# holoskii/Rendering

Measured on AMD Instinct MI355X. Metric: Mrays/s + ms/frame at 4096^2, 250k-tri BVH scene, higher is better.
Workload: dtype f32

## Files before the change

### rendering_amd/csrc/rtx_kernels.hip

```cpp
#include <hip/hip_runtime.h>
#include <stdint.h>

#include "rtx_device.h"
#include "rtx_tuning.h"

#pragma clang fp contract(off)

using namespace rtxd;

constexpr uint32_t kPopNum = 1u, kPopDen = 2u;

namespace {

#if RTX_DBG
#define RTX_DBG_ONLY(...) __VA_ARGS__
#else
#define RTX_DBG_ONLY(...)
#endif
#if RTX_DBG || RTX_WAVE_TRACE
#define RTX_TRACE_ONLY(...) __VA_ARGS__
#else
#define RTX_TRACE_ONLY(...)
#endif

// ... 1094 lines not shown
	s.li = 0; s.si = 0; s.dsum = 0; s.ssum = 0;
}

struct LightRec { int type; V3 color; float intensity; V3 dir, pos; uint32_t nPoints; const float* points; };

template <bool PLAIN = false>
__device__ __forceinline__ void advance(const Params& P, Lane& s, uint32_t gl)
{
	const int maxDepth = P.view.maxDepth;
	const float bias = P.view.bias;
	V3& col = PLAIN ? s.diff : s.col;
	bool run = true;
	do {
		if (!run) continue;
		if (s.state == ST_NEWRAY) {
			RTX_T0
			if (s.sp > maxDepth) { col = skyColor(P, s.rd); s.state = ST_RETURN; RTX_ACC(0) continue; }
			s.qtmax = kFltMax;
			s.state = ST_WAIT_PRIMARY;
			run = false; continue;
		}
		if (s.state == ST_NEXT_LIGHT) {
			RTX_T0
			if (s.li >= P.nLights) { s.state = ST_LIGHTS_DONE; continue; }
			const uint32_t li0 = __builtin_amdgcn_readfirstlane(s.li);
			uint32_t liS = li0;
			if (PLAIN) asm volatile("" : "+s"(liS));
			if (s.li != li0) continue;
			LightRec lr;
			{
				const u32x16 w = sload16(P.lights + liS);
				lr.type = (int)w[0]; lr.color = mk(F(w[1]), F(w[2]), F(w[3])); lr.intensity = F(w[4]);
				lr.dir = mk(F(w[5]), F(w[6]), F(w[7])); lr.pos = mk(F(w[8]), F(w[9]), F(w[10])); lr.nPoints = w[11];
				lr.points = (const float*)(((uint64_t)w[13] << 32) | w[12]);
			}
			const LightRec* l = &lr;
			const int lt = l->type;
			if (PLAIN && lt != 1 && lt != 2) __builtin_unreachable();
			float dist;
			if (lt == 1) {
				s.L = l->dir;
				s.I = l->color * l->intensity;
				dist = kFltMax;
			}
			else if (lt == 2) {
				const V3 lp = l->pos;
				V3 L = s.P - lp;
				s.I = l->color * attenuation(l->intensity, len2(L));
				s.L = normalized(L);
				dist = length(s.P - lp);
			}
			else {
				const uint32_t np = l->nPoints;
				if (s.si == 0) {
					const V3 lp = l->pos;
					s.I = l->color * attenuation(l->intensity, len2(s.P - lp));
					s.dsum = 0; s.ssum = 0;
				}
				if (s.si >= np) {
					const float fn = (float)np;
					if (s.mat == 0) s.diff = s.diff + s.I * (s.dsum / fn);
					else if (s.mat == 3) {
						s.diff = s.diff + s.I * (s.dsum / fn);
						s.spec = s.spec + s.I * powfRef(s.ssum / fn, s.nSpec);
					}
					else s.spec = s.spec + s.I * powfRef(s.ssum / fn, s.nSpec);
					s.li++; s.si = 0;
					continue;
				}
				V3 L = s.P - load3(inGlobal(l->points) + (size_t)s.si * 3);
				dist = length(L);
				s.L = normalized(L);
			}
			s.qmoot = s.mat == 0 && fmaxRef(0.f, dot(s.N, -s.L)) == 0.f;
			s.qarea = lt == 3;
			s.qsrc = (lt == 2 && liS < P.nSrcLights && len2(s.N) <= P.srcNmax2) ? 2u + liS : 0u;
			s.qtmax = dist;
			s.state = ST_WAIT_SHADOW;
			RTX_ACC(1)
			run = false; continue;
		}
		if (s.state == ST_LIGHTS_DONE) {
			RTX_T0
			const Object* ob = P.objects + s.obj;
			if (PLAIN && s.mat != 0) __builtin_unreachable();
			if (s.mat == 0) { col = s.objColor * s.diff; s.state = ST_RETURN; continue; }
			if (s.mat == 3) {
				s.col = s.objColor * ob->ambient + s.diff * ob->diffuse + s.spec * s.specCoef;
				s.state = ST_RETURN; continue;
			}
			if (s.mat == 1) {
				frameAt(P, gl, s.sp, 0) = __int_as_float(FR_REFL);
				frameAt(P, gl, s.sp, 2) = s.spec.x; frameAt(P, gl, s.sp, 3) = s.spec.y; frameAt(P, gl, s.sp, 4) = s.spec.z;
				const V3 nd = s.rd - s.N * (2 * dot(s.rd, s.N));
				s.ro = s.P + s.N * bias; s.rd = nd;
				s.sp++; s.state = ST_NEWRAY; RTX_ACC(2) continue;
			}
			const float ior = ob->ior;
			const float kr = fresnelKr(s.rd, s.N, ior);
			const bool outside = dot(s.rd, s.N) < 0;
			const V3 biasVec = s.N * bias;
			const V3 fd = normalized(reflectDir(s.rd, s.N));
			const V3 fo = outside ? s.P + biasVec : s.P - biasVec;
			frameAt(P, gl, s.sp, 1) = kr;
			frameAt(P, gl, s.sp, 2) = s.spec.x; frameAt(P, gl, s.sp, 3) = s.spec.y; frameAt(P, gl, s.sp, 4) = s.spec.z;
			if (kr < 1) {
				const V3 rd = normalized(refractDir(s.rd, s.N, ior));
				const V3 ro = outside ? s.P - biasVec : s.P + biasVec;
				frameAt(P, gl, s.sp, 0) = __int_as_float(FR_TRANS1);
				frameAt(P, gl, s.sp, 8) = fo.x; frameAt(P, gl, s.sp, 9) = fo.y; frameAt(P, gl, s.sp, 10) = fo.z;
				frameAt(P, gl, s.sp, 11) = fd.x; frameAt(P, gl, s.sp, 12) = fd.y; frameAt(P, gl, s.sp, 13) = fd.z;
				s.ro = ro; s.rd = rd;
			}
			else {
				frameAt(P, gl, s.sp, 0) = __int_as_float(FR_TRANS2);
				frameAt(P, gl, s.sp, 5) = 0.f; frameAt(P, gl, s.sp, 6) = 0.f; frameAt(P, gl, s.sp, 7) = 0.f;
				s.ro = fo; s.rd = fd;
			}
			s.sp++; s.state = ST_NEWRAY; RTX_ACC(3) continue;
		}
		if (s.state == ST_RETURN) {
			RTX_T0
			if (s.sp == 0) { s.state = ST_DONE; run = false; continue; }
			if (PLAIN) __builtin_unreachable();
			s.sp--;
			float fr[kFrameFields];
			for (int k = 0; k < kFrameFields; ++k) fr[k] = frameAt(P, gl, s.sp, k);
			asm volatile("" : "+v"(fr[0]), "+v"(fr[1]), "+v"(fr[2]), "+v"(fr[3]), "+v"(fr[4]), "+v"(fr[5]), "+v"(fr[6]));
			asm volatile("" : "+v"(fr[7]), "+v"(fr[8]), "+v"(fr[9]), "+v"(fr[10]), "+v"(fr[11]), "+v"(fr[12]), "+v"(fr[13]));
			const int kind = __float_as_int(fr[0]);
			const V3 spec = mk(fr[2], fr[3], fr[4]);
			if (kind == FR_REFL) { s.col = s.col * 0.8f + spec; RTX_ACC(4) continue; }
			const float kr = fr[1];
			if (kind == FR_TRANS1) {
				const V3 acc = mk(0, 0, 0) + s.col * (1 - kr);
				frameAt(P, gl, s.sp, 0) = __int_as_float(FR_TRANS2);
				frameAt(P, gl, s.sp, 5) = acc.x; frameAt(P, gl, s.sp, 6) = acc.y; frameAt(P, gl, s.sp, 7) = acc.z;
				s.ro = mk(fr[8], fr[9], fr[10]);
				s.rd = mk(fr[11], fr[12], fr[13]);
				s.sp++; s.state = ST_NEWRAY; RTX_ACC(5) continue;
			}
			V3 acc = mk(fr[5], fr[6], fr[7]);
			acc = acc + s.col * kr;
			s.col = acc + spec * kr;
			RTX_ACC(6)
			continue;
		}
		run = false;
	} while (ballot(run) != 0);
}

template <bool PLAIN = false>
__device__ __forceinline__ void consume(const Params& P, Lane& s, const Hit& h)
{
	if (s.state == ST_WAIT_PRIMARY) {
		RTX_T0
		if (h.obj < 0) { (PLAIN ? s.diff : s.col) = skyColor(P, s.rd); s.state = ST_RETURN; RTX_ACC(7) return; }
		shadePrimary(P, s, h);
		if (PLAIN) s.mat = 0;
		s.state = ST_NEXT_LIGHT;
		RTX_ACC(8)
		return;
	}
	if (s.state == ST_WAIT_SHADOW) {
		RTX_T0
		const float vis = (h.obj < 0) ? 1.0f : 0.0f;
		if (PLAIN && (s.mat != 0 || s.qarea)) __builtin_unreachable();
		const bool area = s.qarea;
		const V3 nL = -s.L;
		if (s.mat == 0) {
			const float c = vis * fmaxRef(0.f, dot(s.N, nL));
			if (!area) s.diff = s.diff + s.I * c;
			else s.dsum += c;
		}
		else {
			const V3 R = reflectDir(s.L, s.N);
			const float sd = fmaxRef(0.f, dot(R, -s.rd));
			if (!area) {
				const V3 vI = s.I * vis;
				if (s.mat == 3) s.diff = s.diff + vI * fmaxRef(0.f, dot(s.N, nL));
				s.spec = s.spec + vI * powfRef(sd, s.nSpec);
			}
			else {
				if (s.mat == 3) s.dsum += vis * fmaxRef(0.f, dot(s.N, nL));
				s.ssum += vis * sd;
			}
		}
		if (area) s.si++; else s.li++;
		s.state = ST_NEXT_LIGHT;
		RTX_ACC(9)
	}
}

__device__ __forceinline__ void primaryRay(const Params& P, float x, float y, V3& o, V3& d)
{
	const float w = (float)P.view.width, hgt = (float)P.view.height;
	const float xp = (2 * (x + 0.5f) / w - 1) * P.view.scale * P.view.aspect;
	const float yp = -(2 * (y + 0.5f) / hgt - 1) * P.view.scale;
	const V3 s = normalized(mk(xp, yp, -1));
	const float* M = P.view.camM;
	V3 r;
	r.x = s.x * M[0] + s.y * M[4] + s.z * M[8] + M[12];
	r.y = s.x * M[1] + s.y * M[5] + s.z * M[9] + M[13];
	r.z = s.x * M[2] + s.y * M[6] + s.z * M[10] + M[14];
	const float ww = s.x * M[3] + s.y * M[7] + s.z * M[11] + M[15];
	if (ww != 0.0f && ww != 1.0f) { const float wi = 1.0f / ww; r.x *= wi; r.y *= wi; r.z *= wi; }
	o = mk(P.view.camPos[0], P.view.camPos[1], P.view.camPos[2]);
	d = r;
}

constexpr int kParkFields = 25;
template <bool PLAIN> struct ParkLayout { static constexpr int kFields = kParkFields - (PLAIN ? 4 : 0), kSp = PLAIN ? -3 : 0; };
template <bool PLAIN>
__device__ __forceinline__ float (*parkArea())[256]
{
	__shared__ float area[ParkLayout<PLAIN>::kFields][256];
	return area;
}
static_assert(sizeof(powTab) + sizeof(leafBatch) + sizeof(wideStack) + sizeof(pruneUni) + ParkLayout<false>::kFields * 1024 <= (RTX_WAVES >= 5 ? 31744 : 40960),
              "the ray kernels' LDS no longer fits the blocks per CU that RTX_WAVES asks for");
static_assert(RTX_WAVES_PLAIN < 6 || sizeof(leafBatch) + sizeof(wideStack) + sizeof(pruneUni) + ParkLayout<true>::kFields * 1024 <= 27136,
              "the PLAIN kernels' LDS no longer fits six blocks per CU (160 KB / 6, rounded down to the allocation granule)");

__device__ __forceinline__ const Params& freshParams(const Params& P)
{
	uint64_t p = (uint64_t)(uintptr_t)__builtin_amdgcn_kernarg_segment_ptr();
	asm volatile("" : "+s"(p));
	return *(const Params*)(const RTX_AS4 Params*)p;
}

template <bool STATS, bool MESH = true, bool FEWRAYS = false, bool BOXES = true, bool CAM = true, int CULLK = -1, bool PLAIN = false>
__device__ __forceinline__ V3 castRayWave(const Params& P0, bool valid, V3 o, V3 d, uint32_t gl, Counts& cnt)
{
	const Params& P = freshParams(P0);
	Lane s;
	s.state = valid ? ST_NEWRAY : ST_DONE;
	s.sp = 0; s.ro = o; s.rd = d; s.col = mk(0, 0, 0);
	s.obj = 0; s.mat = 0; s.li = 0; s.si = 0;
	s.P = s.N = s.objColor = s.diff = s.spec = s.L = s.I = mk(0, 0, 0);
	s.specCoef = s.nSpec = s.dsum = s.ssum = 0;
	s.qtmax = kFltMax; s.qmoot = false; s.qarea = false; s.qsrc = 0;
	RTX_DBG_ONLY(unsigned long long dbgRounds = 0, dbgTrace = 0, dbgState = 0;)
	for (;;) {
		advance<PLAIN>(freshParams(P0), s, gl);
		if (ballot(s.state != ST_DONE) == 0) break;
		Hit h;
		RTX_DBG_ONLY(const unsigned long long dbgT0 = __builtin_readcyclecounter();)
		const bool moot = s.state == ST_WAIT_SHADOW && s.qmoot;
		if (STATS) cnt.moot += __popcll(ballot(moot));
		const bool qshadow = s.state == ST_WAIT_SHADOW;
		const V3 qo = qshadow ? s.P + s.N * P.view.bias : s.ro, qd = qshadow ? -s.L : s.rd;
		const bool qactive = s.state != ST_DONE && (STATS || !moot);
		const float qtmax = s.qtmax;
		const uint32_t qsrc = qshadow ? s.qsrc : ((CAM && s.sp == 0) ? 1u : 0u);
		if (MESH) { s.qtmax = kFltMax; s.qmoot = false; s.qsrc = 0; }
		if (MESH) {
			const uint32_t t = threadIdx.x;
			float (*parkedState)[256] = parkArea<PLAIN>();
			constexpr int kSp = ParkLayout<PLAIN>::kSp;
			parkedState[0][t] = s.P.x; parkedState[1][t] = s.P.y; parkedState[2][t] = s.P.z;
			parkedState[3][t] = s.N.x; parkedState[4][t] = s.N.y; parkedState[5][t] = s.N.z;
			parkedState[6][t] = s.objColor.x; parkedState[7][t] = s.objColor.y; parkedState[8][t] = s.objColor.z;
			parkedState[9][t] = s.diff.x; parkedState[10][t] = s.diff.y; parkedState[11][t] = s.diff.z;
			if (!PLAIN) { parkedState[12][t] = s.spec.x; parkedState[13][t] = s.spec.y; parkedState[14][t] = s.spec.z; }
			parkedState[15 + kSp][t] = s.L.x; parkedState[16 + kSp][t] = s.L.y; parkedState[17 + kSp][t] = s.L.z;
			parkedState[18 + kSp][t] = s.I.x; parkedState[19 + kSp][t] = s.I.y; parkedState[20 + kSp][t] = s.I.z;
			parkedState[21 + kSp][t] = s.rd.x; parkedState[22 + kSp][t] = s.rd.y; parkedState[23 + kSp][t] = s.rd.z;
			if (!PLAIN) parkedState[24][t] = s.specCoef;
			asm volatile("" ::: "memory");
		}
		traceWave<STATS, MESH, FEWRAYS, BOXES, CULLK>(freshParams(P0), qactive, qshadow, qo, qd, qtmax, h, cnt, qsrc);
		if (MESH) {
			asm volatile("" ::: "memory");
			const uint32_t t = threadIdx.x;
			float (*parkedState)[256] = parkArea<PLAIN>();
			constexpr int kSp = ParkLayout<PLAIN>::kSp;
			s.P = mk(parkedState[0][t], parkedState[1][t], parkedState[2][t]);
			s.N = mk(parkedState[3][t], parkedState[4][t], parkedState[5][t]);
			s.objColor = mk(parkedState[6][t], parkedState[7][t], parkedState[8][t]);
			s.diff = mk(parkedState[9][t], parkedState[10][t], parkedState[11][t]);
			if (!PLAIN) s.spec = mk(parkedState[12][t], parkedState[13][t], parkedState[14][t]);
			s.L = mk(parkedState[15 + kSp][t], parkedState[16 + kSp][t], parkedState[17 + kSp][t]);
			s.I = mk(parkedState[18 + kSp][t], parkedState[19 + kSp][t], parkedState[20 + kSp][t]);
			s.rd = mk(parkedState[21 + kSp][t], parkedState[22 + kSp][t], parkedState[23 + kSp][t]);
			if (!PLAIN) s.specCoef = parkedState[24][t];
		}
		RTX_DBG_ONLY(const unsigned long long dbgT1 = __builtin_readcyclecounter();)
		if (s.state != ST_DONE) {
			const Params& Pa = freshParams(P0);
			consume<PLAIN>(Pa, s, h);
		}
		RTX_DBG_ONLY(dbgRounds++; dbgTrace += dbgT1 - dbgT0; dbgState += __builtin_readcyclecounter() - dbgT1;)
	}
	RTX_DBG_ONLY(
	if (__lane_id() == 0) {
		const unsigned long long before = atomicMax(&gDbgHist[8], dbgTrace + dbgState);
		if (dbgTrace + dbgState > before) { gDbgHist[9] = dbgRounds; gDbgHist[10] = dbgTrace; gDbgHist[11] = dbgState; }
		atomicAdd(&gDbgHist[12], dbgRounds); atomicAdd(&gDbgHist[13], dbgTrace); atomicAdd(&gDbgHist[14], dbgState); atomicAdd(&gDbgHist[15], 1ull);
	}
	)
	return PLAIN ? s.diff : s.col;
}

__device__ __forceinline__ bool rowOwned(uint32_t bandH, uint32_t nParts, uint32_t part, uint32_t y)
{
	return bandH == 0 || (y / bandH) % nParts == part;
}
__device__ __forceinline__ bool rowRendered(const Params& P, uint32_t y)
{
	if (rowOwned(P.bandH, P.nParts, P.part, y)) return true;
	if (!P.halo) return false;
	return (y > 0 && rowOwned(P.bandH, P.nParts, P.part, y - 1)) || rowOwned(P.bandH, P.nParts, P.part, y + 1);
}

__device__ __forceinline__ uint32_t nextWork(uint32_t* counter)
{
	uint32_t w = 0;
	if (__lane_id() == 0) w = atomicAdd(counter, 1u);
	return __builtin_amdgcn_readfirstlane(w);
}

__device__ __forceinline__ void flushCounts(const Params& P, const Counts& c)
{
	if (__lane_id() == 0) {
		atomicAdd(P.counters + 0, c.rays);
		atomicAdd(P.counters + 1, c.box);
		atomicAdd(P.counters + 2, c.tri);
		atomicAdd(P.counters + 5, c.wNodes); atomicAdd(P.counters + 6, c.wTri); atomicAdd(P.counters + 7, c.wS2);
		atomicAdd(P.counters + 8, c.wS3); atomicAdd(P.counters + 9, c.wS4);
		atomicAdd(P.counters + 10, c.wLeaves); atomicAdd(P.counters + 11, c.wLeafSkips);
		atomicAdd(P.counters + 12, c.wChunks); atomicAdd(P.counters + 13, c.wChunkSkips); atomicAdd(P.counters + 14, c.triLanes);
		atomicAdd(P.counters + 15, c.moot);
		RTX_DBG_ONLY(
		atomicAdd(&gDbgHist[32], c.cNodes); atomicAdd(&gDbgHist[33], c.cFilter); atomicAdd(&gDbgHist[34], c.cExact);
		atomicAdd(&gDbgHist[40], c.aWalks); atomicAdd(&gDbgHist[41], c.sWalks); atomicAdd(&gDbgHist[42], c.sVisits); atomicAdd(&gDbgHist[43], c.sLeaves); atomicAdd(&gDbgHist[44], c.sPasses); atomicAdd(&gDbgHist[45], c.sExact);
		)
	}
}

}

template <bool STATS, bool MESH = true, bool BOXES = true, int CULLK = (STATS || !MESH) ? -1 : 1, bool PLAIN = false>
__global__ void __launch_bounds__(256, MESH ? (PLAIN ? RTX_WAVES_PLAIN : RTX_WAVES) : RTX_WAVES_ANALYTIC) rtxPass1Kernel(const Params P)
{
	if (!PLAIN) fillPowTab();
	const uint32_t gl = blockIdx.x * blockDim.x + threadIdx.x;
	const uint32_t lane = __lane_id();
	const uint32_t W = P.view.width, H = P.view.height;
	Counts cnt = {};
	const uint32_t xcd = __builtin_amdgcn_s_getreg((3 << 11) | (0 << 6) | 20) & 7u;
	RTX_TRACE_ONLY(
	const unsigned long long dbgStart = wall_clock64();
	unsigned long long dbgEnd = dbgStart, dbgBusy = 0;
	)
	for (uint32_t attempt = 0; attempt < 8; attempt = uni(attempt + 1)) {
		const uint32_t q = (xcd + attempt) & 7u;
		const uint32_t qBase = sload1(P.tileList + q), qSize = sload1(P.tileList + 8 + q);
		uint32_t take = 1, jEnd = 0, j = 0;
		for (;;) {
			if (j >= jEnd) {
				uint32_t w = 0;
				if (__lane_id() == 0) w = atomicAdd(P.workCounter + q * 16, take);
				j = __builtin_amdgcn_readfirstlane(w);
				if (j >= qSize) break;
				jEnd = j + take < qSize ? j + take : qSize;
				if (kPopDen * j >= kPopNum * qSize) take = RTX_POP_MANY;
			}
			const uint32_t tile = sload1(P.tileList + qBase + j);
			j = uni(j + 1);
			RTX_DBG_ONLY(if (P.pad3 != 0 && tile != P.pad3 - 1) continue;)
			uint32_t tx, ty, x, y; bool strip, valid;
			auto place = [&](const Params& Pt, uint32_t ln) {
				strip = (tile & Pt.stripBit) != 0;
				tx = strip ? ((tile >> 16) & 0xfffu) * 8 : tile & 0xffffu; ty = strip ? (tile & 0x7fffu) >> 3 : tile >> 16;
				x = strip ? tx * 8 + ln : tx * 8 + (ln & 7); y = strip ? tile & 0x7fffu : ty * 8 + (ln >> 3);
				valid = x < Pt.view.width - 1 && y < Pt.view.height - 1 && y >= Pt.rowBegin && y < Pt.rowEnd && rowRendered(Pt, y);
			};
			const Params& Pa = freshParams(P);
			place(Pa, laneNow());
			if (ballot(valid) == 0) continue;
			V3 o, d;
			primaryRay(Pa, (float)x + 0.5f, (float)y + 0.5f, o, d);
			if (take > 1) __builtin_amdgcn_s_setprio(0);
			else
			if (sload1(Pa.tileCost + ty * Pa.tilesXFull + tx) > RTX_PRIO_TICKS) __builtin_amdgcn_s_setprio(3); else __builtin_amdgcn_s_setprio(0);
			const unsigned long long t0 = wall_clock64();
			const V3 c = castRayWave<STATS, MESH, false, BOXES, true, CULLK, PLAIN>(Pa, valid, o, d, gl, cnt);
			const unsigned long long dt = wall_clock64() - t0;
			RTX_TRACE_ONLY(dbgEnd = t0 + dt; dbgBusy += dt;)
			uint32_t tileWas = tile;
			asm volatile("" : "+s"(tileWas));
			const Params& Pb = freshParams(P);
			{
				const uint32_t ln = laneNow();
				const bool strip2 = (tileWas & Pb.stripBit) != 0;
				const uint32_t tx2 = strip2 ? ((tileWas >> 16) & 0xfffu) * 8 : tileWas & 0xffffu, ty2 = strip2 ? (tileWas & 0x7fffu) >> 3 : tileWas >> 16;
				const uint32_t x2 = strip2 ? tx2 * 8 + ln : tx2 * 8 + (ln & 7), y2 = strip2 ? tileWas & 0x7fffu : ty2 * 8 + (ln >> 3);
				const bool valid2 = x2 < Pb.view.width - 1 && y2 < Pb.view.height - 1 && y2 >= Pb.rowBegin && y2 < Pb.rowEnd && rowRendered(Pb, y2);
				if (ln == 0) {
					if (!strip2) Pb.tileCost[ty2 * Pb.tilesXFull + tx2] = dt > 0xffffffffull ? 0xffffffffu : (uint32_t)dt;
					if (STATS) { atomicMax(Pb.counters + 3, dt); atomicAdd(Pb.counters + 4, dt); }
				}
				if (strip2 && ln < 8 && tx2 + ln < Pb.tilesX) Pb.tileCost[ty2 * Pb.tilesXFull + tx2 + ln] = (uint32_t)((dt > 0xffffffffull ? 0xffffffffull : dt) / 8);
				if (valid2) {
					float* px = Pb.fb + ((size_t)y2 * Pb.view.width + x2) * 3;
					px[0] = c.x; px[1] = c.y; px[2] = c.z;
				}
			}
		}
	}
	RTX_TRACE_ONLY(if (lane == 0 && (gl >> 6) < 16384) { gDbgWave[3 * (gl >> 6)] = dbgStart; gDbgWave[3 * (gl >> 6) + 1] = dbgEnd; gDbgWave[3 * (gl >> 6) + 2] = dbgBusy; })
	if (STATS || RTX_DBG) flushCounts(P, cnt);
}

__device__ __forceinline__ uint32_t nthSetBit(uint64_t m, uint32_t n)
{
	uint32_t pos = 0;
	uint32_t lo = (uint32_t)m, c = __popc(lo);
	if (n >= c) { pos = 32; n -= c; lo = (uint32_t)(m >> 32); }
	c = __popc(lo & 0xffffu); if (n >= c) { pos += 16; n -= c; lo >>= 16; }
	c = __popc(lo & 0xffu); if (n >= c) { pos += 8; n -= c; lo >>= 8; }
	c = __popc(lo & 0xfu); if (n >= c) { pos += 4; n -= c; lo >>= 4; }
	c = __popc(lo & 0x3u); if (n >= c) { pos += 2; n -= c; lo >>= 2; }
	if (n >= (lo & 1u)) pos += 1;
	return pos;
}

template <bool STATS, bool MESH = true, bool BOXES = true, int CULLK = (STATS || !MESH) ? -1 : 1, bool PLAIN = false>
__global__ void __launch_bounds__(256, MESH ? RTX_WAVES_SSAA : RTX_WAVES_ANALYTIC) rtxSsaaKernel(const Params P)
{
	if (!PLAIN) fillPowTab();
	const uint32_t gl = blockIdx.x * blockDim.x + threadIdx.x;
	const uint32_t lane = __lane_id();
	const uint32_t W = P.view.width, H = P.view.height;
	Counts cnt = {};
	RTX_DBG_ONLY(uint32_t dbgItems = 0;)
	for (;;) {
		const uint32_t work = nextWork(P.workCounter);
		const uint32_t total = sload1(P.ssaaScan + 2 * (size_t)P.nTiles);
		const uint32_t first = work * 16;
		if (first >= total) break;
		if (first < sload1(P.ssaaScan + P.nTiles)) __builtin_amdgcn_s_setprio(3); else __builtin_amdgcn_s_setprio(0);
		const uint32_t g = first + (lane >> 2), sub = lane & 3;
		const uint32_t pxy = P.ssaaPixels[g < total ? g : first];
		const bool valid = g < total && pxy != 0xffffffffu;
		const uint32_t x = pxy & 0xffffu, y = pxy >> 16;
		const float fx = (float)x + ((sub & 2) ? 0.75f : 0.25f), fy = (float)y + ((sub & 1) ? 0.75f : 0.25f);
		V3 o, d;
		primaryRay(P, fx, fy, o, d);
		const unsigned long long t0 = wall_clock64();
		const V3 c = castRayWave<STATS, MESH, true, BOXES, true, CULLK, PLAIN>(P, valid, o, d, gl, cnt);
		if (!STATS) {
			const uint32_t npx = (uint32_t)__popcll(ballot(valid)) >> 2;
			const unsigned long long dt16 = (wall_clock64() - t0) * (npx <= 4u ? 4u : (npx <= 8u ? 2u : 1u));
			if (lane == 0 && pxy != 0xffffffffu) atomicMax(P.tileCost + P.nTiles + (y >> 3) * P.tilesXFull + (x >> 3), (uint32_t)(dt16 > 0xffffffffull ? 0xffffffffull : dt16));
		}
		RTX_DBG_ONLY(
		if (!STATS && lane == 0 && (gl >> 6) < 8192 && dbgItems < 160) {
			const size_t e = (size_t)(gl >> 6) * 160 + dbgItems;
			gDbgTimeline[3 * e] = t0; gDbgTimeline[3 * e + 1] = wall_clock64() - t0; gDbgTimeline[3 * e + 2] = 2ull << 32 | pxy;
		}
		dbgItems++;
		)
		if (STATS && lane == 0) { atomicMax(P.counters + 3, wall_clock64() - t0); atomicAdd(P.counters + 4, wall_clock64() - t0); }
		const int base = (int)(lane & ~3u);
		V3 sum = mk(0, 0, 0);
		for (int k = 0; k < 4; ++k)
			sum = sum + mk(__shfl(c.x, base + k), __shfl(c.y, base + k), __shfl(c.z, base + k));
		if (valid && sub == 0) {
			float* px = P.fb + ((size_t)y * W + x) * 3;
			px[0] = sum.x / 4; px[1] = sum.y / 4; px[2] = sum.z / 4;
		}
	}
	if (STATS || RTX_DBG) flushCounts(P, cnt);
}

__global__ void __launch_bounds__(256) rtxTileListKernel(const uint32_t* __restrict__ plan, uint32_t tilesX, uint32_t nStrips, uint32_t in0, uint32_t in1,
                                                         uint32_t sIn0, uint32_t sIn1, uint32_t* __restrict__ list)
{
	const uint32_t row = blockIdx.y, c = blockIdx.x * blockDim.x + threadIdx.x;
	if (row == 0 && c < 16) list[c] = plan[c];
	const uint32_t kind = plan[16 + 4 * row], val = plan[17 + 4 * row], base0 = plan[18 + 4 * row], base1 = plan[19 + 4 * row];
	const bool inY = (kind & 0x100u) != 0;
	if ((kind & 0xffu) == 1u) {
		if (c >= tilesX) return;
		const uint32_t nIn = inY && in1 > in0 ? in1 - in0 : 0u;
		const bool in = nIn != 0 && c >= in0 && c < in1;
		list[in ? base0 + (c - in0) : base1 + (nIn != 0 && c >= in1 ? c - nIn : c)] = val << 16 | c;
	}
	else if ((kind & 0xffu) == 2u) {
		if (c >= nStrips) return;
		const uint32_t nIn = inY && sIn1 > sIn0 ? sIn1 - sIn0 : 0u;
		const bool in = nIn != 0 && c >= sIn0 && c < sIn1;
		list[in ? base0 + (c - sIn0) : base1 + (nIn != 0 && c >= sIn1 ? c - nIn : c)] = 0x10000000u | c << 16 | val;
	}
}

__global__ void __launch_bounds__(256) rtxTileMarkKernel(const uint32_t* __restrict__ list, uint32_t tilesXFull, uint8_t* __restrict__ mark)
{
	const uint32_t q = blockIdx.y, base = list[q], n = list[8 + q];
	for (uint32_t i = blockIdx.x * blockDim.x + threadIdx.x; i < n; i += gridDim.x * blockDim.x) {
		const uint32_t t = list[base + i];
		mark[(t >> 16) * tilesXFull + (t & 0xffffu)] = 1;
	}
}

__global__ void __launch_bounds__(256) rtxTileNeedKernel(const uint8_t* __restrict__ mark, uint32_t tilesXFull, uint32_t tilesYFull,
                                                         uint8_t* __restrict__ need, uint32_t* __restrict__ expect, uint32_t* __restrict__ blocksDone)
{
	const uint32_t t = blockIdx.x * blockDim.x + threadIdx.x;
	if (t < tilesXFull * tilesYFull) {
		uint32_t n = 0;
		if (mark[t]) {
			const int ty = (int)(t / tilesXFull), tx = (int)(t - (uint32_t)ty * tilesXFull);
			for (int dy = -1; dy <= 1; ++dy)
				for (int dx = -1; dx <= 1; ++dx) {
					const int x = tx + dx, y = ty + dy;
					if (x >= 0 && y >= 0 && x < (int)tilesXFull && y < (int)tilesYFull) n += mark[(uint32_t)y * tilesXFull + (uint32_t)x];
				}
			atomicAdd(expect + (t & 63u), 1u);
		}
		need[t] = (uint8_t)n;
	}
	__syncthreads();
	if (threadIdx.x == 0) {
		__threadfence();
		if (atomicAdd(blocksDone, 1u) + 1 == gridDim.x) {
			uint32_t groups = 0;
			for (int k = 0; k < 64; ++k) groups += atomicAdd(expect + k, 0u) != 0;
			expect[64] = groups;
		}
	}
}

__global__ void __launch_bounds__(256) rtxFrameClearKernel(uint32_t* __restrict__ work, uint32_t* __restrict__ deps, size_t depWords,
                                                           uint32_t* __restrict__ ctl, uint32_t ctlWords, uint32_t errWord, uint8_t* __restrict__ mask, size_t maskBytes)
{
	const size_t t = (size_t)blockIdx.x * blockDim.x + threadIdx.x, stride = (size_t)gridDim.x * blockDim.x;
	if (t < 2) work[16 + t] = 0;
	if (t < 128) work[128 + t] = 0;
	for (size_t i = t; i < ctlWords; i += stride) { if (i == errWord && ctl[i]) work[24] = ctl[i]; ctl[i] = 0; }
	for (size_t i = t; i < depWords; i += stride) deps[i] = 0;
	for (size_t i = t; i < maskBytes; i += stride) mask[i] = 0;
}

struct SplatSources { uint32_t n; int32_t kind[16]; uint32_t weight[16]; float l[16][3]; float p[16][6]; };
__global__ void __launch_bounds__(256) rtxCostSplatKernel(const float* __restrict__ boxes, uint32_t nLeaves, const View view, uint32_t gridW, uint32_t gridH,
                                                          uint32_t* __restrict__ grid, const SplatSources src)
{
	const uint32_t i = blockIdx.x * blockDim.x + threadIdx.x;
	if (i >= nLeaves) return;
	const float* b = boxes + (size_t)i * 8;
	const uint32_t sIdx = blockIdx.y;
	const uint32_t wgt = sIdx != 0 ? src.weight[sIdx - 1] : 1u;
	const uint32_t n = (uint32_t)b[6] * wgt;
	const float* M = view.camM;
	float x0 = 1e30f, x1 = -1e30f, y0 = 1e30f, y1 = -1e30f;
	for (int c = 0; c < 8; ++c) {
		float cx = b[(c & 1) ? 3 : 0], cy = b[(c & 2) ? 4 : 1], cz = b[(c & 4) ? 5 : 2];
		if (sIdx != 0) {
			const uint32_t k = sIdx - 1;
			const bool point = src.kind[k] == 2;
			const float dx = point ? cx - src.l[k][0] : src.l[k][0], dy = point ? cy - src.l[k][1] : src.l[k][1], dz = point ? cz - src.l[k][2] : src.l[k][2];
			const float nx = src.p[k][3], ny = src.p[k][4], nz = src.p[k][5];
			const float den = dx * nx + dy * ny + dz * nz;
			if (!(fabsf(den) > 1e-6f)) return;
			const float t = ((src.p[k][0] - cx) * nx + (src.p[k][1] - cy) * ny + (src.p[k][2] - cz) * nz) / den;
			if (!(t > 0.0f) || !(t < 1e4f)) return;
			cx += t * dx; cy += t * dy; cz += t * dz;
		}
		const float px = cx - view.camPos[0], py = cy - view.camPos[1], pz = cz - view.camPos[2];
		const float sx = px * M[0] + py * M[1] + pz * M[2], sy = px * M[4] + py * M[5] + pz * M[6], sz = px * M[8] + py * M[9] + pz * M[10];
		if (!(sz < -1e-4f)) return;
		const float xp = sx / -sz, yp = sy / -sz;
		const float fx = (xp / (view.scale * view.aspect) + 1.0f) * 0.5f * (float)view.width - 1.0f, fy = (-yp / view.scale + 1.0f) * 0.5f * (float)view.height - 1.0f;
		x0 = fminf(x0, fx); x1 = fmaxf(x1, fx); y0 = fminf(y0, fy); y1 = fmaxf(y1, fy);
	}
	if (!(x1 >= 0.0f && y1 >= 0.0f && x0 < (float)view.width && y0 < (float)view.height)) return;
	const int cx0 = max(0, (int)floorf(x0 / 16.0f)), cx1 = min((int)gridW - 1, (int)floorf(x1 / 16.0f));
	const int cy0 = max(0, (int)floorf(y0 / 16.0f)), cy1 = min((int)gridH - 1, (int)floorf(y1 / 16.0f));
	if ((long long)(cx1 - cx0 + 1) * (cy1 - cy0 + 1) > 4096) return;
	for (int cy = cy0; cy <= cy1; ++cy)
		for (int cx = cx0; cx <= cx1; ++cx)
			atomicAdd((unsigned long long*)(grid + 2 * ((size_t)cy * gridW + cx)), ((unsigned long long)wgt << 32) | n);
}

struct FarPlanes { float p[4][6]; uint32_t n; float farDist; uint32_t farTicks; };
__global__ void __launch_bounds__(256) rtxCostFillKernel(const uint32_t* __restrict__ grid, uint32_t gridW, uint32_t tilesXFull, uint32_t tilesYFull,
                                                         uint32_t* __restrict__ tileCost, float perRef, float perLeaf, float base, const View view, const FarPlanes far)
{
	const uint32_t t = blockIdx.x * blockDim.x + threadIdx.x;
	if (t >= tilesXFull * tilesYFull) return;
	const uint32_t ty = t / tilesXFull, tx = t - ty * tilesXFull;
	const size_t cell = (size_t)(ty / 2) * gridW + tx / 2;
	const float refs = (float)grid[2 * cell], leaves = (float)grid[2 * cell + 1];
	uint32_t c = leaves > 0 ? (uint32_t)fminf(base + perRef * refs + perLeaf * leaves, 4.0e9f) : 0u;
	if (far.n) {
		const float* M = view.camM;
		for (int k = 0; k < 2; ++k) {
			const float x = (float)(tx * 8 + 4) + 0.5f, y = (float)(ty * 8 + (k ? 7 : 0)) + 0.5f;
			const float xp = (2 * (x + 0.5f) / (float)view.width - 1) * view.scale * view.aspect, yp = -(2 * (y + 0.5f) / (float)view.height - 1) * view.scale;
			const float il = rsqrtf(xp * xp + yp * yp + 1.0f);
			const float sx = xp * il, sy = yp * il, sz = -il;
			const float dx = sx * M[0] + sy * M[4] + sz * M[8], dy = sx * M[1] + sy * M[5] + sz * M[9], dz = sx * M[2] + sy * M[6] + sz * M[10];
			for (uint32_t q = 0; q < far.n; ++q) {
				const float den = dx * far.p[q][3] + dy * far.p[q][4] + dz * far.p[q][5];
				if (!(fabsf(den) > 1e-12f)) continue;
				const float tt = ((far.p[q][0] - view.camPos[0]) * far.p[q][3] + (far.p[q][1] - view.camPos[1]) * far.p[q][4] + (far.p[q][2] - view.camPos[2]) * far.p[q][5]) / den;
				if (tt > far.farDist) c = max(c, far.farTicks);
			}
		}
	}
	tileCost[t] = c;
}

__global__ void __launch_bounds__(256) rtxTileClassKernel(const uint32_t* __restrict__ cost, uint32_t tilesXFull, uint32_t tilesYFull,
                                                          uint8_t* __restrict__ klass, unsigned long long* __restrict__ costSum)
{
	const uint32_t t = blockIdx.x * blockDim.x + threadIdx.x;
	{
		unsigned long long mine = t < tilesXFull * tilesYFull ? cost[t] : 0;
		for (int sh = 32; sh > 0; sh >>= 1) mine += __shfl_xor(mine, sh);
		if ((threadIdx.x & 63) == 0 && mine) atomicAdd(costSum, mine);
	}
	if (t >= tilesXFull * tilesYFull) return;
	const int ty = (int)(t / tilesXFull), tx = (int)(t - (uint32_t)ty * tilesXFull);
	uint32_t c = 0;
	for (int dy = -2; dy <= 2; ++dy)
		for (int dx = -2; dx <= 2; ++dx) {
			const int x = tx + dx, y = ty + dy;
			if (x >= 0 && y >= 0 && x < (int)tilesXFull && y < (int)tilesYFull) c = max(c, cost[(uint32_t)y * tilesXFull + (uint32_t)x]);
		}
	klass[t] = (uint8_t)(c ? 31u - (uint32_t)__builtin_clz(c) : 0u);
}

template <bool PLACE>
__global__ void __launch_bounds__(256) rtxTileOrderKernel(uint32_t* __restrict__ global, const uint32_t* __restrict__ list, const uint32_t* __restrict__ cost,
                                                           uint32_t tilesXFull, uint32_t* __restrict__ out, const uint8_t* __restrict__ klassIn = nullptr,
                                                           const unsigned long long* __restrict__ costSum = nullptr, uint32_t nWaves = 1,
                                                           uint32_t splitPercent = 0, uint32_t splitFloor = 0, uint32_t* __restrict__ thresholds = nullptr,
                                                           uint32_t tilesX = 0, uint32_t stripLimit = 0xffffffffu, uint32_t* __restrict__ heads = nullptr,
                                                           uint32_t stripBit = 0)
{
	if (PLACE && heads && blockIdx.x == 0 && blockIdx.y == 0 && threadIdx.x < 128) heads[threadIdx.x] = 0;
	uint32_t split4 = 0xffffffffu, split16 = 0xffffffffu;
	if (costSum && splitPercent) {
		const unsigned long long even = *costSum / nWaves * splitPercent / 100;
		split4 = even > 0x0fffffffull ? 0x0fffffffu : (uint32_t)even;
		if (split4 < splitFloor) split4 = splitFloor;
		split16 = split4 * 4;
	}
	__shared__ uint32_t hist[32], cursor[32];
	const uint32_t q = blockIdx.y;
	const uint32_t base = list[q], n = list[8 + q];
	const uint32_t obase = 16 + 16 * (base - 16);
	if (threadIdx.x < 32) hist[threadIdx.x] = 0;
	if (thresholds && q == 0 && blockIdx.x == 0 && threadIdx.x == 0) { thresholds[0] = split4; thresholds[1] = split16; }
	__syncthreads();
	auto entry = [&](uint32_t tile) {
		return (tile & stripBit) ? ((tile & 0x7fffu) >> 3) * tilesXFull + ((tile >> 16) & 0xfffu) * 8 : (tile >> 16) * tilesXFull + (tile & 0xffffu);
	};
	auto klass = [&](uint32_t tile) {
		if (klassIn) return (uint32_t)klassIn[entry(tile)];
		uint32_t c = cost[entry(tile)];
		if (tile & stripBit) c = c > 0x1fffffffu ? 0xffffffffu : c * 8;
		return c ? 31u - (uint32_t)__builtin_clz(c) : 0u;
	};
	auto parts = [&](uint32_t tile) {
		if (tile & stripBit) {
			const uint32_t tx0 = ((tile >> 16) & 0xfffu) * 8, n = tilesX - tx0 < 8u ? tilesX - tx0 : 8u;
			unsigned long long sum = 0;
			for (uint32_t e = 0; e < n; ++e) sum += cost[entry(tile) + e];
			return sum > stripLimit ? n : 1u;
		}
		const uint32_t c = cost[entry(tile)];
		return c > split16 ? 16u : (c > split4 ? 4u : 1u);
	};
	const uint32_t piece = (n + gridDim.x - 1) / gridDim.x, i0 = blockIdx.x * piece, i1 = i0 + piece < n ? i0 + piece : n;
	if (!PLACE) {
		for (uint32_t i = i0 + threadIdx.x; i < i1; i += blockDim.x) { const uint32_t tile = list[base + i]; atomicAdd(&hist[klass(tile)], parts(tile)); }
		__syncthreads();
		if (threadIdx.x < 32) global[(q * 32 + blockIdx.x) * 32 + threadIdx.x] = hist[threadIdx.x];
		return;
	}
	if (gridDim.x == 1) {
		for (uint32_t i = i0 + threadIdx.x; i < i1; i += blockDim.x) { const uint32_t tile = list[base + i]; atomicAdd(&hist[klass(tile)], parts(tile)); }
		__syncthreads();
		if (threadIdx.x == 0) {
			uint32_t run = 0;
			for (int k = 31; k >= 0; k--) { cursor[k] = run; run += hist[k]; }
// ... 691 lines not shown
```

### rendering_amd/csrc/rtx_rays.hip

```cpp
#pragma clang fp contract(off)

namespace {

constexpr int kRayKeyBits = 30;

__device__ __forceinline__ uint32_t orderedBits(float f)
{
	const uint32_t u = __float_as_uint(f);
	return (u & 0x80000000u) ? ~u : (u | 0x80000000u);
}
__device__ __forceinline__ float orderedFloat(uint32_t u) { return __uint_as_float((u & 0x80000000u) ? (u & 0x7fffffffu) : ~u); }

struct RayAxes { float m[9]; float cam[3]; };
__device__ __forceinline__ void octahedral(const RayAxes& ax, float dx, float dy, float dz, float& u, float& v)
{
	const float x = dx * ax.m[0] + dy * ax.m[1] + dz * ax.m[2];
	const float y = dx * ax.m[3] + dy * ax.m[4] + dz * ax.m[5];
	const float z = dx * ax.m[6] + dy * ax.m[7] + dz * ax.m[8];
	const float l1 = fabsf(x) + fabsf(y) + fabsf(z);
	u = x / l1; v = y / l1;
	if (z > 0) {
		const float fu = (1.0f - fabsf(v)) * (u < 0 ? -1.0f : 1.0f), fv = (1.0f - fabsf(u)) * (v < 0 ? -1.0f : 1.0f);
		u = fu; v = fv;
	}
}

__device__ __forceinline__ void rayCoords(const float* ray, const RayAxes& ax, float c[5])
{
	octahedral(ax, ray[3], ray[4], ray[5], c[0], c[1]);
	const float ox = ray[0] - ax.cam[0], oy = ray[1] - ax.cam[1], oz = ray[2] - ax.cam[2];
	octahedral(ax, ox, oy, oz, c[2], c[3]);
	c[4] = __builtin_log2f(fabsf(ox) + fabsf(oy) + fabsf(oz));
}

__device__ __forceinline__ float waveMinF(float v)
{
	for (int k = 32; k >= 1; k >>= 1) v = fminf(v, __shfl_xor(v, k));
	return v;
}
__device__ __forceinline__ float waveMaxF(float v)
{
	for (int k = 32; k >= 1; k >>= 1) v = fmaxf(v, __shfl_xor(v, k));
	return v;
}

}

__global__ void __launch_bounds__(256) rtxRayBoxKernel(const float* rays, uint32_t n, RayAxes ax, uint32_t* box, double* spread)
{
	float lo[5], hi[5];
	double sp[5];
	for (int k = 0; k < 5; k++) { lo[k] = __builtin_inff(); hi[k] = -__builtin_inff(); sp[k] = 0.0; }
	const uint32_t groups = (uint32_t)(((size_t)n + 63) / 64), waves = gridDim.x * 4;
	for (uint32_t g = blockIdx.x * 4 + (threadIdx.x >> 6); g < groups; g += waves) {
		const size_t i = (size_t)g * 64 + __lane_id();
		float c[5] = { 0, 0, 0, 0, 0 };
		const bool valid = i < n;
		if (valid) rayCoords(rays + i * 6, ax, c);
		for (int k = 0; k < 5; k++) {
			const bool fin = valid && fabsf(c[k]) < __builtin_inff();
			const float a = waveMinF(fin ? c[k] : __builtin_inff()), b = waveMaxF(fin ? c[k] : -__builtin_inff());
			if (a <= b) { lo[k] = fminf(lo[k], a); hi[k] = fmaxf(hi[k], b); sp[k] += (double)b - (double)a; }
		}
	}
	__shared__ float part[2][5][4];
	__shared__ double partSp[5][4];
	const uint32_t w = threadIdx.x >> 6;
	if (__lane_id() == 0) for (int k = 0; k < 5; k++) { part[0][k][w] = lo[k]; part[1][k][w] = hi[k]; partSp[k][w] = sp[k]; }
	__syncthreads();
	if (threadIdx.x < 5) {
		const int k = threadIdx.x;
		const float a = fminf(fminf(part[0][k][0], part[0][k][1]), fminf(part[0][k][2], part[0][k][3]));
		const float b = fmaxf(fmaxf(part[1][k][0], part[1][k][1]), fmaxf(part[1][k][2], part[1][k][3]));
		if (a <= b) {
			atomicMin(box + k, orderedBits(a)); atomicMax(box + 5 + k, orderedBits(b));
			atomicAdd(spread + k, (partSp[k][0] + partSp[k][1]) + (partSp[k][2] + partSp[k][3]));
		}
	}
}

__global__ void __launch_bounds__(256) rtxRayKeyKernel(const float* rays, uint32_t n, RayAxes ax, const uint32_t* box, const double* spread,
                                                       int originFirst, int check, uint32_t* keys)
{
	const size_t i = (size_t)blockIdx.x * blockDim.x + threadIdx.x;
	if (i >= n) return;
	int dims[5], nd = 0;
	float base[5], scale[5];
	double haveO = 0, haveD = 0;
	int nO = 0, nD = 0;
	const double groups = (double)(((size_t)n + 63) / 64);
	for (int j = 0; j < 5; j++) {
		const int k = originFirst ? (j + 2) % 5 : j;
		const float a = orderedFloat(box[k]), b = orderedFloat(box[5 + k]);
		if (!(b > a) || !(b - a < __builtin_inff())) continue;
		base[nd] = a; scale[nd] = 1.0f / (b - a); dims[nd] = k; nd++;
		const double have = spread[k] / groups / ((double)b - (double)a);
		if (k >= 2) { haveO += have; nO++; } else { haveD += have; nD++; }
	}
	uint32_t key = 0;
	const bool keep = check && nd > 0 && (nO ? haveO / nO : haveD / nD) <= exp2(log2(64.0 / (double)n) / nd);
	if (nd > 0 && !keep) {
		float c[5];
		rayCoords(rays + i * 6, ax, c);
		const int per = kRayKeyBits / nd;
		uint32_t q[5];
		for (int j = 0; j < nd; j++) {
			const float f = fminf(fmaxf((c[dims[j]] - base[j]) * scale[j], 0.0f), 1.0f) * (float)(1u << per);
			q[j] = min((uint32_t)f, (1u << per) - 1u);
		}
		for (int b = per - 1; b >= 0; b--)
			for (int j = 0; j < nd; j++) key = key << 1 | ((q[j] >> b) & 1u);
		key <<= kRayKeyBits - per * nd;
	}
	keys[i] = key;
}

namespace {

__device__ __forceinline__ void loadRay(const Params& P, const uint32_t* order, uint32_t k, bool valid, uint32_t& i, V3& o, V3& d)
{
	i = valid ? (order ? order[k] : k) : 0u;
	o = mk(0, 0, 0); d = mk(0, 0, -1);
	if (valid) { o = load3(P.probeRays + (size_t)i * 6); d = load3(P.probeRays + (size_t)i * 6 + 3); }
}

__device__ __forceinline__ void storeHit(const Params& P, const Hit& h, float* out)
{
	const bool hit = h.obj >= 0;
	const bool mesh = hit && P.objects[hit ? h.obj : 0].type == 3;
	out[0] = hit ? 1.f : 0.f; out[1] = hit ? (float)h.obj : -1.f; out[2] = mesh ? (float)h.tri : -1.f;
	out[3] = h.t; out[4] = hit ? h.u : -1.f; out[5] = hit ? h.v : -1.f; out[6] = 0; out[7] = 0;
}

}

template <bool MESH, bool BOXES, int CULLK>
__global__ void __launch_bounds__(256) rtxRayHitKernel(const Params P, const uint32_t* order, float* hits)
{
	const uint32_t lane = __lane_id();
	const uint32_t nWork = (P.nProbe + 63) / 64;
	Counts cnt = {};
	for (;;) {
		const uint32_t work = nextWork(P.workCounter);
		if (work >= nWork) break;
		const uint32_t k = work * 64 + lane;
		const bool valid = k < P.nProbe;
		uint32_t i; V3 o, d;
		loadRay(P, order, k, valid, i, o, d);
		Hit h;
		traceWave<false, MESH, false, BOXES, CULLK>(P, valid, false, o, d, kFltMax, h, cnt);
		if (valid) storeHit(P, h, hits + (size_t)i * 8);
	}
}

template <bool MESH, bool BOXES, int CULLK, bool ORDER>
__global__ void __launch_bounds__(256) rtxRayOccludedKernel(const Params P, const uint32_t* order, const float* tmax, uint8_t* occluded)
{
	const uint32_t lane = __lane_id();
	const uint32_t nWork = (P.nProbe + 63) / 64;
	Counts cnt = {};
	for (;;) {
		const uint32_t work = nextWork(P.workCounter);
		if (work >= nWork) break;
		const uint32_t k = work * 64 + lane;
		const bool valid = k < P.nProbe;
		uint32_t i; V3 o, d;
		loadRay(P, order, k, valid, i, o, d);
		const float tm = (valid && tmax) ? tmax[i] : __builtin_inff();
		const bool asked = valid && !(tm != tm);
		bool open = asked;
		Hit h;
		const float tmWalk = tm > kFltMax ? kFltMax : tm;
		if (!MESH) {
			traceWave<false, false, false, BOXES, CULLK>(P, open, true, o, d, tm, h, cnt);
			open = open && h.obj < 0;
		}
		else if (ORDER) {
			traceWave<false, true, false, BOXES, CULLK>(P, open, true, o, d, tmWalk, h, cnt);
			open = open && h.obj < 0;
			if (ballot(open && tm > kFltMax) != 0) {
				traceWave<false, false, false, BOXES, CULLK, 1>(P, open && tm > kFltMax, true, o, d, tm, h, cnt);
				open = open && h.obj < 0;
			}
		}
		else {
			traceWave<false, false, false, BOXES, CULLK, 1>(P, open, true, o, d, tm, h, cnt);
			open = open && h.obj < 0;
			if (ballot(open) != 0) {
				traceWave<false, true, false, BOXES, CULLK, 2>(P, open, true, o, d, tmWalk, h, cnt);
				open = open && h.obj < 0;
			}
		}
		if (valid) occluded[i] = (asked && !open) ? 1 : 0;
	}
}

template <bool MESH, bool BOXES, int CULLK, bool PLAIN>
__global__ void __launch_bounds__(256, MESH ? (PLAIN ? RTX_WAVES_PLAIN : RTX_WAVES) : RTX_WAVES_ANALYTIC) rtxRayColourKernel(const Params P, const uint32_t* order, float* colours)
{
	if (!PLAIN) fillPowTab();
	const uint32_t gl = blockIdx.x * blockDim.x + threadIdx.x;
	const uint32_t lane = __lane_id();
	const uint32_t nWork = (P.nProbe + 63) / 64;
	Counts cnt = {};
	for (;;) {
		const uint32_t work = nextWork(P.workCounter);
		if (work >= nWork) break;
		const uint32_t k = work * 64 + lane;
		const bool valid = k < P.nProbe;
		uint32_t i; V3 o, d;
		loadRay(P, order, k, valid, i, o, d);
		const V3 c = castRayWave<false, MESH, false, BOXES, false, CULLK, PLAIN>(P, valid, o, d, gl, cnt);
		if (valid) { float* pc = colours + (size_t)i * 3; pc[0] = c.x; pc[1] = c.y; pc[2] = c.z; }
	}
}

__global__ void __launch_bounds__(256) rtxRayNormalsKernel(const Params P, const uint32_t* order, float* hits, float* colours)
{
	const uint32_t lane = __lane_id();
	const uint32_t nWork = (P.nProbe + 63) / 64;
	for (;;) {
		const uint32_t work = nextWork(P.workCounter);
		if (work >= nWork) break;
		const uint32_t k = work * 64 + lane;
		const bool valid = k < P.nProbe;
		uint32_t i; V3 o, d;
		loadRay(P, order, k, valid, i, o, d);
		Hit h;
		const V3 c = normalsCast(P, valid, o, d, 0u, h);
		if (valid && hits) storeHit(P, h, hits + (size_t)i * 8);
		if (valid && colours) { float* pc = colours + (size_t)i * 3; pc[0] = c.x; pc[1] = c.y; pc[2] = c.z; }
	}
}

template __global__ void rtxRayHitKernel<true, true, 1>(const Params, const uint32_t*, float*);
template __global__ void rtxRayHitKernel<true, false, 1>(const Params, const uint32_t*, float*);
template __global__ void rtxRayHitKernel<true, true, 0>(const Params, const uint32_t*, float*);
template __global__ void rtxRayHitKernel<true, false, 0>(const Params, const uint32_t*, float*);
template __global__ void rtxRayHitKernel<false, true, -1>(const Params, const uint32_t*, float*);
#define RTX_RAY_COLOUR_INSTANCES(PL)                                                                         \
template __global__ void rtxRayColourKernel<true, true, 1, PL>(const Params, const uint32_t*, float*);     \
template __global__ void rtxRayColourKernel<true, false, 1, PL>(const Params, const uint32_t*, float*);    \
template __global__ void rtxRayColourKernel<true, true, 0, PL>(const Params, const uint32_t*, float*);     \
template __global__ void rtxRayColourKernel<true, false, 0, PL>(const Params, const uint32_t*, float*);
RTX_RAY_COLOUR_INSTANCES(false) RTX_RAY_COLOUR_INSTANCES(true)
#undef RTX_RAY_COLOUR_INSTANCES
template __global__ void rtxRayColourKernel<false, true, -1, false>(const Params, const uint32_t*, float*);
#define RTX_RAY_OCCLUDED_INSTANCES(ORD)                                                                                       \
template __global__ void rtxRayOccludedKernel<true, true, 1, ORD>(const Params, const uint32_t*, const float*, uint8_t*);   \
template __global__ void rtxRayOccludedKernel<true, false, 1, ORD>(const Params, const uint32_t*, const float*, uint8_t*);  \
template __global__ void rtxRayOccludedKernel<true, true, 0, ORD>(const Params, const uint32_t*, const float*, uint8_t*);   \
template __global__ void rtxRayOccludedKernel<true, false, 0, ORD>(const Params, const uint32_t*, const float*, uint8_t*);
RTX_RAY_OCCLUDED_INSTANCES(false) RTX_RAY_OCCLUDED_INSTANCES(true)
#undef RTX_RAY_OCCLUDED_INSTANCES
template __global__ void rtxRayOccludedKernel<false, true, -1, true>(const Params, const uint32_t*, const float*, uint8_t*);

__global__ void __launch_bounds__(64) rtxRayInitKernel(uint32_t* work)
{
	const uint32_t t = threadIdx.x;
	if (t < 54) work[t] = (t >= 32 && t < 37) ? ~0u : 0u;
}
```

Measured before the change: 17760.

## Add straight-line PLAIN cast path that parks live shading state in LDS

For the PLAIN (diffuse-only) pass, the generic state-machine ray caster is replaced by a straight-line routine that traces the primary ray, then one shadow ray per light. Live shading values (direction, origin, hit point, normal, colour, accumulated diffuse, light intensity) are written to a 16-field per-thread shared-memory area around each traversal and read back afterwards. The aim is to cut register pressure and state-machine overhead during BVH traversal and so keep or raise wave occupancy. In exchange it adds LDS traffic and 16 KB of LDS per block, guarded by a static_assert so six blocks still fit per CU.

```diff
diff --git a/rendering_amd/csrc/rtx_kernels.hip b/rendering_amd/csrc/rtx_kernels.hip
--- a/rendering_amd/csrc/rtx_kernels.hip
+++ b/rendering_amd/csrc/rtx_kernels.hip
@@ -1420,6 +1420,94 @@
 	return PLAIN ? s.diff : s.col;
 }
 
+constexpr int kParkFieldsPlainWave = 16;
+__device__ __forceinline__ float (*parkAreaPlainWave())[256]
+{
+	__shared__ float area[kParkFieldsPlainWave][256];
+	return area;
+}
+static_assert(RTX_WAVES_PLAIN < 6 || sizeof(leafBatch) + sizeof(wideStack) + sizeof(pruneUni) + kParkFieldsPlainWave * 1024 <= 27136,
+              "the PLAIN pass-1 kernel's LDS no longer fits six blocks per CU");
+
+template <bool STATS, bool FEWRAYS = false, bool BOXES = true, bool CAM = true, int CULLK = -1>
+__device__ __forceinline__ V3 castRayPlainWave(const Params& P0, bool valid, V3 o, V3 d, uint32_t gl, Counts& cnt)
+{
+	static_assert(!STATS, "the instrumented kernels count moot rays and rounds: they keep the state machine (castRayWave)");
+	const uint32_t t = threadIdx.x;
+	float (*parked)[256] = parkAreaPlainWave();
+	Lane s;
+	s.diff = mk(0, 0, 0);
+	if (freshParams(P0).view.maxDepth < 0) {
+		if (valid) s.diff = skyColor(freshParams(P0), d);
+		return s.diff;
+	}
+	Hit h;
+	parked[0][t] = d.x; parked[1][t] = d.y; parked[2][t] = d.z;
+	if (!CAM) { parked[3][t] = o.x; parked[4][t] = o.y; parked[5][t] = o.z; }
+	asm volatile("" ::: "memory");
+	traceWave<STATS, true, FEWRAYS, BOXES, CULLK>(freshParams(P0), valid, false, o, d, kFltMax, h, cnt, CAM ? 1u : 0u);
+	asm volatile("" ::: "memory");
+	const bool hit = h.obj >= 0;
+	{
+		const Params& P = freshParams(P0);
+		s.rd = mk(parked[0][t], parked[1][t], parked[2][t]);
+		s.ro = CAM ? mk(P.view.camPos[0], P.view.camPos[1], P.view.camPos[2]) : mk(parked[3][t], parked[4][t], parked[5][t]);
+		if (valid && !hit) s.diff = skyColor(P, s.rd);
+		if (ballot(hit) == 0) return s.diff;
+		s.P = s.N = s.objColor = mk(0, 0, 0);
+		if (hit) shadePrimary(P, s, h);
+	}
+	for (uint32_t li = 0; li < uni(freshParams(P0).nLights); li = uni(li + 1)) {
+		V3 I; float m;
+		{
+			const Params& P = freshParams(P0);
+			const u32x16 w = sload16(P.lights + li);
+			const int lt = (int)w[0];
+			const V3 lcolor = mk(F(w[1]), F(w[2]), F(w[3])); const float lint = F(w[4]);
+			V3 L; float dist;
+			if (lt == 1) {
+				L = mk(F(w[5]), F(w[6]), F(w[7]));
+				I = lcolor * lint;
+				dist = kFltMax;
+			}
+			else {
+				const V3 lp = mk(F(w[8]), F(w[9]), F(w[10]));
+				const V3 Lv = s.P - lp;
+				I = lcolor * attenuation(lint, len2(Lv));
+				L = normalized(Lv);
+				dist = length(s.P - lp);
+			}
+			const V3 nL = -L;
+			m = fmaxRef(0.f, dot(s.N, nL));
+			const bool active = hit && !(m == 0.f);
+			h.obj = -1;
+			if (ballot(active) != 0) {
+				const uint32_t src = (lt == 2 && li < P.nSrcLights && len2(s.N) <= P.srcNmax2) ? 2u + li : 0u;
+				const V3 so = s.P + s.N * P.view.bias;
+				parked[0][t] = s.P.x; parked[1][t] = s.P.y; parked[2][t] = s.P.z;
+				parked[3][t] = s.N.x; parked[4][t] = s.N.y; parked[5][t] = s.N.z;
+				parked[6][t] = s.objColor.x; parked[7][t] = s.objColor.y; parked[8][t] = s.objColor.z;
+				parked[9][t] = s.diff.x; parked[10][t] = s.diff.y; parked[11][t] = s.diff.z;
+				parked[12][t] = I.x; parked[13][t] = I.y; parked[14][t] = I.z;
+				parked[15][t] = m;
+				asm volatile("" ::: "memory");
+				traceWave<STATS, true, FEWRAYS, BOXES, CULLK>(freshParams(P0), active, true, so, nL, dist, h, cnt, src);
+				asm volatile("" ::: "memory");
+				s.P = mk(parked[0][t], parked[1][t], parked[2][t]);
+				s.N = mk(parked[3][t], parked[4][t], parked[5][t]);
+				s.objColor = mk(parked[6][t], parked[7][t], parked[8][t]);
+				s.diff = mk(parked[9][t], parked[10][t], parked[11][t]);
+				I = mk(parked[12][t], parked[13][t], parked[14][t]);
+				m = parked[15][t];
+			}
+		}
+		const float vis = (h.obj < 0) ? 1.0f : 0.0f;
+		const float c = vis * m;
+		if (hit) s.diff = s.diff + I * c;
+	}
+	return hit ? s.objColor * s.diff : s.diff;
+}
+
 __device__ __forceinline__ bool rowOwned(uint32_t bandH, uint32_t nParts, uint32_t part, uint32_t y)
 {
 	return bandH == 0 || (y / bandH) % nParts == part;
@@ -1503,7 +1591,9 @@
 			else
 			if (sload1(Pa.tileCost + ty * Pa.tilesXFull + tx) > RTX_PRIO_TICKS) __builtin_amdgcn_s_setprio(3); else __builtin_amdgcn_s_setprio(0);
 			const unsigned long long t0 = wall_clock64();
-			const V3 c = castRayWave<STATS, MESH, false, BOXES, true, CULLK, PLAIN>(Pa, valid, o, d, gl, cnt);
+			V3 c;
+			if constexpr (PLAIN) c = castRayPlainWave<STATS, false, BOXES, true, CULLK>(Pa, valid, o, d, gl, cnt);
+			else c = castRayWave<STATS, MESH, false, BOXES, true, CULLK, PLAIN>(Pa, valid, o, d, gl, cnt);
 			const unsigned long long dt = wall_clock64() - t0;
 			RTX_TRACE_ONLY(dbgEnd = t0 + dt; dbgBusy += dt;)
 			uint32_t tileWas = tile;
diff --git a/rendering_amd/csrc/rtx_rays.hip b/rendering_amd/csrc/rtx_rays.hip
--- a/rendering_amd/csrc/rtx_rays.hip
+++ b/rendering_amd/csrc/rtx_rays.hip
@@ -210,7 +210,9 @@
 		const bool valid = k < P.nProbe;
 		uint32_t i; V3 o, d;
 		loadRay(P, order, k, valid, i, o, d);
-		const V3 c = castRayWave<false, MESH, false, BOXES, false, CULLK, PLAIN>(P, valid, o, d, gl, cnt);
+		V3 c;
+		if constexpr (PLAIN) c = castRayPlainWave<false, false, BOXES, false, CULLK>(P, valid, o, d, gl, cnt);
+		else c = castRayWave<false, MESH, false, BOXES, false, CULLK, PLAIN>(P, valid, o, d, gl, cnt);
 		if (valid) { float* pc = colours + (size_t)i * 3; pc[0] = c.x; pc[1] = c.y; pc[2] = c.z; }
 	}
 }
```

After: 18210 (median of 6 runs). 2.6% higher.
